# DIAGNijmegen/bodyct-dram-emph-subtype

Measured on AMD Instinct MI355X. Metric: CT volumes/sec (train step, 1x128x256x256), higher is better.
Workload: dtype f32; 1 GPU; BASELINE configs[1]: resnet18segcls train step (fwd+loss+bwd+Adam), batch 2/GPU, 1x128x256x256, fp32, inputs resident in HBM; global_batch=2, parallelism=dp1, hip_graph=False, streams=2

## Files before the change

### bodyct-dram-emph-subtype_amd/csrc/wino_gemm.hip

```cpp
#include <stdlib.h>
#include "wino_gemm.h"

namespace {

template <int MI, int NJ>
__device__ __forceinline__ void zero_acc(f32x16 (&acc)[MI][NJ]) {
#pragma unroll
  for (int mi = 0; mi < MI; ++mi)
#pragma unroll
    for (int nj = 0; nj < NJ; ++nj)
#pragma unroll
      for (int e = 0; e < 16; ++e) acc[mi][nj][e] = 0.f;
}


struct NnTile { const float* Ab; const float* Bb; float* Yb; int mt, nt; };
template <int NJ>
__device__ __forceinline__ NnTile nn_tile(const int idx, const float* A, const float* Bw, float* Y, const int N,
                                          const int K, const int m_tiles, const int n_tiles, const int nblk,
                                          const int npts) {
  constexpr int BN = 64 * NJ;
  const int L = xcd_remap(idx, nblk);
  NnTile t;
  t.nt = L % n_tiles;
// ... 252 lines not shown
            if (fused) {
              v += bv;
              if (ep.add) {
                const long oo = o - Y;
                const f32x4 av = *reinterpret_cast<const f32x4*>(ep.add + oo);
                if (ep.gate) {
                  const f32x4 gv = *reinterpret_cast<const f32x4*>(ep.gate + oo);
#pragma unroll
                  for (int j = 0; j < 4; ++j) v[j] += gv[j] > 0.f ? av[j] : 0.f;
                } else {
                  v += av;
                }
              }
#pragma unroll
              for (int j = 0; j < 4; ++j) { s1v[cr][j] += v[j]; s2v[cr][j] += v[j] * v[j]; }
            }
            *reinterpret_cast<f32x4*>(o) = v;
          }
        }
      }
    }
    if (ep.stats) {
#pragma unroll
      for (int cr = 0; cr < NR; ++cr)
#pragma unroll
        for (int j = 0; j < 4; ++j)
#pragma unroll
          for (int o = Q; o < 64; o <<= 1) {
            s1v[cr][j] += __shfl_xor(s1v[cr][j], o, 64);
            s2v[cr][j] += __shfl_xor(s2v[cr][j], o, 64);
          }
      __syncthreads();
      float* red = s1;
      if (rs == 0) {
#pragma unroll
        for (int cr = 0; cr < NR; ++cr)
#pragma unroll
          for (int j = 0; j < 4; ++j) {
            red[(ln.wave * 2 + 0) * 32 * NJ + cr * CW + 4 * cq + j] = s1v[cr][j];
            red[(ln.wave * 2 + 1) * 32 * NJ + cr * CW + 4 * cq + j] = s2v[cr][j];
          }
      }
      __syncthreads();
      if (ln.tid < 2 * BN) {
        const int which = ln.tid / BN, cc = ln.tid - which * BN;
        const int cwn = cc / (32 * NJ), c2 = cc - cwn * 32 * NJ;
        float v = 0.f;
#pragma unroll
        for (int w = 0; w < 4; ++w) v += red[((cwn * 4 + w) * 2 + which) * 32 * NJ + c2];
        ep.stats[((long)cur.mt * 2 + which) * N + cur.nt * BN + cc] = v;
      }
    }
    if (!more) break;
    idx = nxt;
    cur = nx;
  }
}
#ifndef DRAM_STREAM_NT
#define DRAM_STREAM_NT 2
#endif
template <int NJ, int KT, int S, bool DB = false, int KH = 1>
__global__ __launch_bounds__(256, DB ? 2 : 1) void wino_gemm_nn_stream_kernel(const float* __restrict__ A,
                                                                    const float* __restrict__ Bw, float* __restrict__ Y,
                                                                    const int npts, const int m64, const int per_wg,
                                                                    const int total) {
  constexpr int N = 64 * NJ;
  constexpr int STG = 64 * KT;
  constexpr int SPR = KT / 4;
  constexpr int RPI = 64 / SPR;
  constexpr int IPW = 64 / RPI / 4;
  constexpr int BPW = N / RPI / 4;
  constexpr int KG = KT / 8;
  constexpr int P = DB ? 40 : 32 * NJ + 8;
  constexpr int KS = KT * KH;
  static_assert(S == 3 || S == 4, "ring depth");
  static_assert(KH == 1 || (KH == 2 && DB && S == 3), "k halves: direct-B form, three stages");
  __shared__ __attribute__((aligned(1024))) float st0[STG], st1[STG], st2[STG], st3[S == 4 ? STG : 64];
  __shared__ __attribute__((aligned(1024))) float bt[DB ? 64 : N * KT];
  __shared__ __attribute__((aligned(16))) float turn[4 * 32 * P];

  const int tid = threadIdx.x, lane = tid & 63;
  const int wave = __builtin_amdgcn_readfirstlane(tid >> 6);
  const int li = lane & 31, lh = lane >> 5;
  const int i0 = blockIdx.x * per_wg;
  const int n = (i0 + per_wg <= total ? per_wg : total - i0);
  if (n <= 0) return;

  int aoff[IPW], boff[BPW];
#pragma unroll
  for (int j = 0; j < IPW; ++j) {
    const int row = RPI * (wave + 4 * j) + lane / SPR, ph = lane % SPR;
    aoff[j] = row * KS + ((ph & ~15) | ((ph ^ row) & 15)) * 4;
  }
#pragma unroll
  for (int j = 0; j < BPW; ++j) {
    const int row = RPI * (wave + 4 * j) + lane / SPR, ph = lane % SPR;
    boff[j] = row * KT + ((ph & ~15) | ((ph ^ row) & 15)) * 4;
  }
  auto a_src = [&](int item) __attribute__((always_inline)) {
    const int ti = item / KH, h = item - ti * KH;
    const int xi = ti / m64, t = ti - xi * m64;
    return A + (((long)(t >> 2) * npts + xi) * 256 + (t & 3) * 64) * KS + h * KT;
  };
  auto issue_a = [&](int item, float* stage) __attribute__((always_inline)) {
    const float* src = a_src(item);
#pragma unroll
    for (int j = 0; j < IPW; ++j)
      __builtin_amdgcn_global_load_lds((const __attribute__((address_space(1))) void*)(src + aoff[j]),
                                       (__attribute__((address_space(3))) void*)(stage + (wave + 4 * j) * 256), 16, 0,
                                       DRAM_STREAM_NT);
  };
  auto stage_of = [&](int k) __attribute__((always_inline)) -> float* {
    return k == 0 ? st0 : (k == 1 ? st1 : (k == 2 ? st2 : st3));
  };

  const int r0 = 32 * (wave & 1), c0 = 32 * NJ * (wave >> 1);
  const int arow = r0 + li;
  f32x4 bfr[NJ][KG * KH];
  auto load_b = [&](int xi) __attribute__((always_inline)) {
    if (DB) {
      const float* srcd = Bw + (long)xi * N * KS;
#pragma unroll
      for (int nj = 0; nj < NJ; ++nj)
#pragma unroll
        for (int kg = 0; kg < KG * KH; ++kg)
          bfr[nj][kg] = *reinterpret_cast<const f32x4*>(srcd + (c0 + nj * 32 + li) * KS + (2 * kg + lh) * 4);
      __builtin_amdgcn_s_waitcnt(0x0F70);
      asm volatile("" ::: "memory");
      return;
    }
    __syncthreads();
    const float* src = Bw + (long)xi * N * KT;
#pragma unroll
    for (int j = 0; j < BPW; ++j)
      __builtin_amdgcn_global_load_lds((const __attribute__((address_space(1))) void*)(src + boff[j]),
                                       (__attribute__((address_space(3))) void*)(bt + (wave + 4 * j) * 256), 16, 0, 0);
    __builtin_amdgcn_s_waitcnt(0x0F70);
    asm volatile("" ::: "memory");
    __syncthreads();
#pragma unroll
    for (int nj = 0; nj < NJ; ++nj) {
      const int brow = c0 + nj * 32 + li;
#pragma unroll
      for (int kg = 0; kg < KG; ++kg) {
        const int sl = 2 * kg + lh;
        bfr[nj][kg] = *reinterpret_cast<const f32x4*>(bt + brow * KT + ((sl & ~15) | ((sl ^ brow) & 15)) * 4);
      }
    }
  };

  int xi_cur = i0 / KH / m64;
#pragma unroll
  for (int k = 0; k < S - 1; ++k)
    if (k < n) issue_a(i0 + k, stage_of(k));
  load_b(xi_cur);

  float* reg = turn + wave * (32 * P);
  constexpr int Q = 8 * NJ;
  const int cq = lane % Q, rs = lane / Q;

  constexpr int U = S * KH;
  f32x16 acc[NJ];
  for (int itb = 0; itb < n; itb += U) {
#pragma unroll
    for (int k = 0; k < U; ++k) {
      const int it = itb + k;
      const int h = k % KH;
      if (it < n) {
        const int item = i0 + it;
        const int ti = item / KH;
        const int xi = ti / m64, t = ti - xi * m64;
        if (h == 0 && xi != xi_cur) {
          xi_cur = xi;
          load_b(xi);
        }
        if (it + S - 2 < n) __builtin_amdgcn_s_waitcnt(0x0F70 | ((IPW * (S - 2)) & 15) | (((IPW * (S - 2)) >> 4) << 14));
        else __builtin_amdgcn_s_waitcnt(0x0F70);
        asm volatile("" ::: "memory");
        __builtin_amdgcn_s_barrier();
        if (it + S - 1 < n) issue_a(item + S - 1, stage_of((k + S - 1) % S));
        const float* stg = stage_of(k % S);
        if (h == 0) {
#pragma unroll
          for (int nj = 0; nj < NJ; ++nj)
#pragma unroll
            for (int e = 0; e < 16; ++e) acc[nj][e] = 0.f;
        }
#pragma unroll
        for (int kg = 0; kg < KG; ++kg) {
          const int sl = 2 * kg + lh;
          const f32x4 af = *reinterpret_cast<const f32x4*>(stg + arow * KT + ((sl & ~15) | ((sl ^ arow) & 15)) * 4);
#pragma unroll
          for (int e = 0; e < 4; ++e)
#pragma unroll
            for (int nj = 0; nj < NJ; ++nj)
              acc[nj] = __builtin_amdgcn_mfma_f32_32x32x2f32(af[e], bfr[nj][h * KG + kg][e], acc[nj], 0, 0, 0);
        }
        if (h != KH - 1) continue;
        float* yb = Y + (((long)(t >> 2) * npts + xi) * 256 + (t & 3) * 64 + r0) * N + c0;
        if (DB) {
          const int cq8 = lane & 7, rs8 = lane >> 3;
#pragma unroll
          for (int nj = 0; nj < NJ; ++nj) {
#pragma unroll
            for (int e = 0; e < 16; ++e) reg[((e & 3) + 8 * (e >> 2) + 4 * lh) * P + li] = acc[nj][e];
#pragma unroll
            for (int r = 0; r < 4; ++r) {
              const int row = r * 8 + rs8;
              *reinterpret_cast<f32x4*>(yb + (long)row * N + nj * 32 + 4 * cq8) =
                  *reinterpret_cast<const f32x4*>(reg + row * P + 4 * cq8);
            }
          }
        } else {
#pragma unroll
          for (int e = 0; e < 16; ++e)
#pragma unroll
            for (int nj = 0; nj < NJ; ++nj) reg[((e & 3) + 8 * (e >> 2) + 4 * lh) * P + nj * 32 + li] = acc[nj][e];
#pragma unroll
          for (int r = 0; r < Q / 2; ++r) {
            const int row = r * (64 / Q) + rs;
            *reinterpret_cast<f32x4*>(yb + (long)row * N + 4 * cq) = *reinterpret_cast<const f32x4*>(reg + row * P + 4 * cq);
          }
        }
      }
    }
  }
}

typedef __bf16 bf16x8 __attribute__((ext_vector_type(8)));

template <int NJ, int NT>
__global__ __launch_bounds__(512) void wino_gemm_nn_bf16_kernel(const float* __restrict__ A, const float* __restrict__ Bw,
                                                                float* __restrict__ Y, const int Mpad, const int N,
                                                                const int K, const int m_tiles, const int n_tiles,
                                                                const int nblk, const int npts) {
  constexpr int STAGE = (256 + 64 * NJ) * 32;
  __shared__ __attribute__((aligned(1024))) float lds[2 * STAGE];
  const int tid = threadIdx.x;
  const int lane = tid & 63;
  const int wave = __builtin_amdgcn_readfirstlane(tid >> 6);
  const NnTile t = nn_tile<NJ>(blockIdx.x, A, Bw, Y, N, K, m_tiles, n_tiles, nblk, npts);
  const NnDma<NJ> dma(lane, wave, K);
  const int niter = K / 32;
  f32x16 acc[2][NJ];
  zero_acc(acc);

  const int li = lane & 31, lh = lane >> 5;
  const int wm = wave & 3, wn = wave >> 2;
  const int rsw = (li >> 1) & 7;
  const int a_row = (wm * 64 + li) * 32;
  const int b_row = 256 * 32 + (wn * NJ * 32 + li) * 32;

  dma.issue(t.Ab, t.Bb, 0, lds);
  for (int it = 0; it < niter; ++it) {
    __syncthreads();
    if (it + 1 < niter) dma.issue(t.Ab, t.Bb, it + 1, lds + ((it + 1) & 1) * STAGE);
    const float* st = lds + (it & 1) * STAGE;
#pragma unroll
    for (int j = 0; j < 2; ++j) {
      const int sh = ((2 * j + lh) ^ rsw) * 4, sl = ((4 + 2 * j + lh) ^ rsw) * 4;
      bf16x8 ah[2], al[2], bh[NJ], bl[NJ];
#pragma unroll
      for (int mi = 0; mi < 2; ++mi) {
        ah[mi] = *reinterpret_cast<const bf16x8*>(st + a_row + mi * 32 * 32 + sh);
        if (NT > 1) al[mi] = *reinterpret_cast<const bf16x8*>(st + a_row + mi * 32 * 32 + sl);
      }
#pragma unroll
      for (int nj = 0; nj < NJ; ++nj) {
        bh[nj] = *reinterpret_cast<const bf16x8*>(st + b_row + nj * 32 * 32 + sh);
        if (NT > 1) bl[nj] = *reinterpret_cast<const bf16x8*>(st + b_row + nj * 32 * 32 + sl);
      }
#pragma unroll
      for (int nj = 0; nj < NJ; ++nj)
#pragma unroll
        for (int mi = 0; mi < 2; ++mi) {
          if (NT > 1) {
            acc[mi][nj] = __builtin_amdgcn_mfma_f32_32x32x16_bf16(al[mi], bh[nj], acc[mi][nj], 0, 0, 0);
            acc[mi][nj] = __builtin_amdgcn_mfma_f32_32x32x16_bf16(ah[mi], bl[nj], acc[mi][nj], 0, 0, 0);
          }
          acc[mi][nj] = __builtin_amdgcn_mfma_f32_32x32x16_bf16(ah[mi], bh[nj], acc[mi][nj], 0, 0, 0);
        }
    }
  }

#pragma unroll
  for (int mi = 0; mi < 2; ++mi)
#pragma unroll
    for (int e = 0; e < 16; ++e) {
      const int row = wm * 64 + mi * 32 + (e & 3) + 8 * (e >> 2) + 4 * lh;
      float* o = t.Yb + (long)row * N + wn * NJ * 32 + li;
#pragma unroll
      for (int nj = 0; nj < NJ; ++nj) o[nj * 32] = acc[mi][nj][e];
    }
}

struct TnTile {
  int nt, mt, split, xi;
  int t0, t1;
  __device__ __forceinline__ long row(const int it, const int npts) const {
    const int tt = t0 + it * 32;
    return ((long)(tt >> 8) * npts + xi) * 256 + (tt & 255);
  }
};
__device__ __forceinline__ TnTile tn_tile(const int bid, const int nblk, const int m_tiles, const int n_tiles,
                                          const int nsplit, const int kper, const int Tpad) {
  int L = xcd_remap(bid, nblk);
  TnTile t;
  t.nt = L % n_tiles; L /= n_tiles;
  t.mt = L % m_tiles; L /= m_tiles;
  t.split = L % nsplit;
  t.xi = L / nsplit;
  t.t0 = t.split * kper;
  t.t1 = (t.t0 + kper < Tpad) ? t.t0 + kper : Tpad;
  return t;
}
template <int WMW, int MI, int NJ>
__global__ __launch_bounds__(512) void wino_gemm_tn_kernel(const float* __restrict__ Ah, const float* __restrict__ Bh,
                                                           float* __restrict__ slab, const int Tpad, const int M,
                                                           const int N, const int m_tiles, const int n_tiles,
                                                           const int nsplit, const int kper, const int nblk,
                                                           const int npts) {
  constexpr int WNW = 8 / WMW;
  constexpr int BM = WMW * 32 * MI, BN = WNW * 32 * NJ;
  static_assert(BM % 64 == 0 && BM <= 256 && BN % 64 == 0 && BN <= 256, "one DMA piece = 256 floats");
  constexpr int STAGE = 32 * (BM + BN);
  constexpr int AQ = BM / 4, ARPP = 64 / AQ, APW = BM / 64;
  constexpr int BQ = BN / 4, BRPP = 64 / BQ, BPW = BN / 64;
  __shared__ __attribute__((aligned(1024))) float lds[2 * STAGE];

  const int tid = threadIdx.x;
  const int lane = tid & 63;
  const int wave = __builtin_amdgcn_readfirstlane(tid >> 6);
  const TnTile t = tn_tile(blockIdx.x, nblk, m_tiles, n_tiles, nsplit, kper, Tpad);
  int bcol = t.nt * BN + (lane % BQ) * 4;
  if (bcol > N - 4) bcol = N - 4;
  const float* Ab = Ah + (long)(lane / AQ) * M + t.mt * BM + (lane % AQ) * 4;
  const float* Bb = Bh + (long)(lane / BQ) * N + bcol;

  auto issue = [&](int it, int stage) __attribute__((always_inline)) {
    float* as = lds + stage * STAGE;
    float* bs = as + 32 * BM;
    const long row = t.row(it, npts);
    const float* ag = Ab + row * M;
    const float* bg = Bb + row * N;
#pragma unroll
    for (int j = 0; j < APW; ++j) {
      const int p = APW * wave + j;
      __builtin_amdgcn_global_load_lds((const __attribute__((address_space(1))) void*)(ag + (long)(p * ARPP) * M),
                                       (__attribute__((address_space(3))) void*)(as + p * 256), 16, 0, 0);
    }
#pragma unroll
    for (int jj = 0; jj < BPW; ++jj) {
      const int p = BPW * wave + jj;
      __builtin_amdgcn_global_load_lds((const __attribute__((address_space(1))) void*)(bg + (long)(p * BRPP) * N),
                                       (__attribute__((address_space(3))) void*)(bs + p * 256), 16, 0, 0);
    }
  };

  f32x16 acc[MI][NJ];
  zero_acc(acc);

  const int li = lane & 31, lh = lane >> 5;
  const int wm = wave % WMW, wn = wave / WMW;
  const int niter = (t.t1 - t.t0) / 32;

  if (niter > 0) issue(0, 0);
  for (int it = 0; it < niter; ++it) {
    __syncthreads();
    if (it + 1 < niter) issue(it + 1, (it + 1) & 1);
    const float* as = lds + (it & 1) * STAGE + wm * 32 * MI + li;
    const float* bs = lds + (it & 1) * STAGE + 32 * BM + wn * 32 * NJ + li;
#pragma unroll 4
    for (int kk = 0; kk < 16; ++kk) {
      const int kr = 2 * kk + lh;
      float af[MI], bf[NJ];
#pragma unroll
      for (int mi = 0; mi < MI; ++mi) af[mi] = as[kr * BM + mi * 32];
#pragma unroll
      for (int nj = 0; nj < NJ; ++nj) bf[nj] = bs[kr * BN + nj * 32];
#pragma unroll
      for (int nj = 0; nj < NJ; ++nj)
#pragma unroll
        for (int mi = 0; mi < MI; ++mi)
          acc[mi][nj] = __builtin_amdgcn_mfma_f32_32x32x2f32(af[mi], bf[nj], acc[mi][nj], 0, 0, 0);
    }
  }

  float* sb = slab + (((long)t.split * npts + t.xi) * M + t.mt * BM) * N + t.nt * BN;
#pragma unroll
  for (int mi = 0; mi < MI; ++mi)
#pragma unroll
    for (int e = 0; e < 16; ++e) {
      const int row = wm * 32 * MI + mi * 32 + (e & 3) + 8 * (e >> 2) + 4 * lh;
      float* o = sb + (long)row * N + wn * 32 * NJ + li;
#pragma unroll
      for (int nj = 0; nj < NJ; ++nj)
        if (t.nt * BN + wn * 32 * NJ + nj * 32 + li < N) o[nj * 32] = acc[mi][nj][e];
    }
}

__global__ __launch_bounds__(512, 2) void wino_gemm_tn64_kernel(const float* __restrict__ Ah, const float* __restrict__ Bh,
                                                                float* __restrict__ slab, const int Tpad, const int nsplit,
                                                                const int kper, const int nblk, const int npts) {
  constexpr int M = 64, N = 64, KS = 64;
  constexpr int STAGE = KS * (M + N);
  __shared__ __attribute__((aligned(1024))) float lds[2 * STAGE];
  const int tid = threadIdx.x, lane = tid & 63;
  const int wave = __builtin_amdgcn_readfirstlane(tid >> 6);
  int L = xcd_remap(blockIdx.x, nblk);
  const int split = L % nsplit;
  const int xi = L / nsplit;
  const int t0 = split * kper;
  const int t1 = (t0 + kper < Tpad) ? t0 + kper : Tpad;
  const int prow = lane >> 4, pcol = (lane & 15) * 4;
  auto issue = [&](int it, int stage) __attribute__((always_inline)) {
    float* as = lds + stage * STAGE;
    float* bs = as + KS * M;
    const int tt = t0 + it * KS;
    const long row = ((long)(tt >> 8) * npts + xi) * 256 + (tt & 255);
#pragma unroll
    for (int j = 0; j < 2; ++j) {
      const int p = 2 * wave + j;
      __builtin_amdgcn_global_load_lds((const __attribute__((address_space(1))) void*)(Ah + (row + p * 4 + prow) * M + pcol),
                                       (__attribute__((address_space(3))) void*)(as + p * 256), 16, 0, 0);
      __builtin_amdgcn_global_load_lds((const __attribute__((address_space(1))) void*)(Bh + (row + p * 4 + prow) * N + pcol),
                                       (__attribute__((address_space(3))) void*)(bs + p * 256), 16, 0, 0);
    }
  };
  f32x16 acc;
#pragma unroll
  for (int e = 0; e < 16; ++e) acc[e] = 0.f;
  const int li = lane & 31, lh = lane >> 5;
  const int wm = wave & 1, wn = (wave >> 1) & 1, kh = wave >> 2;
  const int niter = (t1 - t0) / KS;
  if (niter > 0) issue(0, 0);
  for (int it = 0; it < niter; ++it) {
    __syncthreads();
    if (it + 1 < niter) issue(it + 1, (it + 1) & 1);
    const float* as = lds + (it & 1) * STAGE + (kh * 32) * M + wm * 32 + li;
    const float* bs = lds + (it & 1) * STAGE + KS * M + (kh * 32) * N + wn * 32 + li;
#pragma unroll 4
    for (int kk = 0; kk < 16; ++kk) {
      const int kr = 2 * kk + lh;
      acc = __builtin_amdgcn_mfma_f32_32x32x2f32(as[kr * M], bs[kr * N], acc, 0, 0, 0);
    }
  }
  __syncthreads();
  float* ex = lds + (wave & 3) * 1024;
  if (kh == 1) {
#pragma unroll
    for (int e = 0; e < 16; ++e) ex[e * 64 + lane] = acc[e];
  }
  __syncthreads();
  if (kh == 0) {
    float* sb = slab + (((long)split * npts + xi) * M) * N;
#pragma unroll
    for (int e = 0; e < 16; ++e) {
      const int row = wm * 32 + (e & 3) + 8 * (e >> 2) + 4 * lh;
      sb[(long)row * N + wn * 32 + li] = acc[e] + ex[e * 64 + lane];
    }
  }
}

typedef short s16x4 __attribute__((ext_vector_type(4)));
typedef short s16x8 __attribute__((ext_vector_type(8)));

template <int WMW, int MI, int NJ, int NT>
__global__ __launch_bounds__(512) void wino_gemm_tn_bf16_kernel(const float* __restrict__ Ah, const float* __restrict__ Bh,
                                                                float* __restrict__ slab, const int Tpad, const int M,
                                                                const int N, const int m_tiles, const int n_tiles,
                                                                const int nsplit, const int kper, const int nblk,
                                                                const int npts) {
  constexpr int WNW = 8 / WMW;
  constexpr int BM = WMW * 32 * MI, BN = WNW * 32 * NJ;
  static_assert(BM % 64 == 0 && BM <= 256 && BN % 64 == 0 && BN <= 256, "one DMA piece = 256 floats");
  constexpr int STAGE = 32 * (BM + BN);
  constexpr int AQ = BM / 4, ARPP = 64 / AQ, APW = BM / 64;
  constexpr int BQ = BN / 4, BRPP = 64 / BQ, BPW = BN / 64;
  __shared__ __attribute__((aligned(1024))) float lds[2 * STAGE];

  const int tid = threadIdx.x;
  const int lane = tid & 63;
  const int wave = __builtin_amdgcn_readfirstlane(tid >> 6);
  const TnTile t = tn_tile(blockIdx.x, nblk, m_tiles, n_tiles, nsplit, kper, Tpad);

  int acol[APW], bcol[BPW];
#pragma unroll
  for (int j = 0; j < APW; ++j) {
    const int r3 = (j * ARPP + lane / AQ) & 3, slot = lane % AQ;
    acol[j] = t.mt * BM + ((((slot >> 2) ^ r3) << 2) | (slot & 3)) * 4;
  }
#pragma unroll
  for (int j = 0; j < BPW; ++j) {
    const int r3 = (j * BRPP + lane / BQ) & 3, slot = lane % BQ;
    int c = t.nt * BN + ((((slot >> 2) ^ r3) << 2) | (slot & 3)) * 4;
    bcol[j] = c > N - 4 ? N - 4 : c;
  }
  const float* Ab = Ah + (long)(lane / AQ) * M;
  const float* Bb = Bh + (long)(lane / BQ) * N;

  auto issue = [&](int it, int stage) __attribute__((always_inline)) {
    float* as = lds + stage * STAGE;
    float* bs = as + 32 * BM;
    const long row = t.row(it, npts);
    const float* ag = Ab + row * M;
    const float* bg = Bb + row * N;
#pragma unroll
    for (int j = 0; j < APW; ++j) {
      const int p = APW * wave + j;
      __builtin_amdgcn_global_load_lds((const __attribute__((address_space(1))) void*)(ag + (long)(p * ARPP) * M + acol[j]),
                                       (__attribute__((address_space(3))) void*)(as + p * 256), 16, 0, 0);
    }
#pragma unroll
    for (int jj = 0; jj < BPW; ++jj) {
      const int p = BPW * wave + jj;
      __builtin_amdgcn_global_load_lds((const __attribute__((address_space(1))) void*)(bg + (long)(p * BRPP) * N + bcol[jj]),
                                       (__attribute__((address_space(3))) void*)(bs + p * 256), 16, 0, 0);
    }
  };

  f32x16 acc[MI][NJ];
  zero_acc(acc);

  const int li = lane & 31, lh = lane >> 5;
  const int wm = wave % WMW, wn = wave / WMW;
  const int niter = (t.t1 - t.t0) / 32;

  const int g4 = lane >> 4, q = (lane >> 2) & 3, p4 = lane & 3;
  const int rrow = (g4 >> 1) * 8 + q;
  const int cbyte = (g4 & 1) * 32 + p4 * 8;
  int a_hi[MI], a_lo[MI], b_hi[NJ], b_lo[NJ];
#pragma unroll
  for (int mi = 0; mi < MI; ++mi) {
    const int ch = 2 * (wm * MI + mi);
    a_hi[mi] = rrow * BM * 4 + ((ch ^ q) * 64) + cbyte;
    a_lo[mi] = rrow * BM * 4 + (((ch + 1) ^ q) * 64) + cbyte;
  }
#pragma unroll
  for (int nj = 0; nj < NJ; ++nj) {
    const int ch = 2 * (wn * NJ + nj);
    b_hi[nj] = 32 * BM * 4 + rrow * BN * 4 + ((ch ^ q) * 64) + cbyte;
    b_lo[nj] = 32 * BM * 4 + rrow * BN * 4 + (((ch + 1) ^ q) * 64) + cbyte;
  }
  auto frag = [&](const char* st, int off, int rstride) __attribute__((always_inline)) {
    const s16x4 r0 = __builtin_amdgcn_ds_read_tr16_b64_v4i16((__attribute__((address_space(3))) s16x4*)(st + off));
    const s16x4 r1 =
        __builtin_amdgcn_ds_read_tr16_b64_v4i16((__attribute__((address_space(3))) s16x4*)(st + off + 4 * rstride));
    return __builtin_bit_cast(bf16x8, __builtin_shufflevector(r0, r1, 0, 1, 2, 3, 4, 5, 6, 7));
  };

  if (niter > 0) issue(0, 0);
  for (int it = 0; it < niter; ++it) {
    __syncthreads();
    if (it + 1 < niter) issue(it + 1, (it + 1) & 1);
    const char* st = reinterpret_cast<const char*>(lds + (it & 1) * STAGE);
#pragma unroll
    for (int s16 = 0; s16 < 2; ++s16) {
      bf16x8 ah[MI], al[MI], bh[NJ], bl[NJ];
#pragma unroll
      for (int mi = 0; mi < MI; ++mi) {
        ah[mi] = frag(st, a_hi[mi] + s16 * 16 * BM * 4, BM * 4);
        if (NT > 1) al[mi] = frag(st, a_lo[mi] + s16 * 16 * BM * 4, BM * 4);
      }
#pragma unroll
      for (int nj = 0; nj < NJ; ++nj) {
        bh[nj] = frag(st, b_hi[nj] + s16 * 16 * BN * 4, BN * 4);
        if (NT > 1) bl[nj] = frag(st, b_lo[nj] + s16 * 16 * BN * 4, BN * 4);
      }
#pragma unroll
      for (int nj = 0; nj < NJ; ++nj)
#pragma unroll
        for (int mi = 0; mi < MI; ++mi) {
          if (NT > 1) {
            acc[mi][nj] = __builtin_amdgcn_mfma_f32_32x32x16_bf16(al[mi], bh[nj], acc[mi][nj], 0, 0, 0);
            acc[mi][nj] = __builtin_amdgcn_mfma_f32_32x32x16_bf16(ah[mi], bl[nj], acc[mi][nj], 0, 0, 0);
          }
          acc[mi][nj] = __builtin_amdgcn_mfma_f32_32x32x16_bf16(ah[mi], bh[nj], acc[mi][nj], 0, 0, 0);
        }
    }
  }

  float* sb = slab + (((long)t.split * npts + t.xi) * M + t.mt * BM) * N + t.nt * BN;
#pragma unroll
  for (int mi = 0; mi < MI; ++mi)
#pragma unroll
    for (int e = 0; e < 16; ++e) {
      const int row = wm * 32 * MI + mi * 32 + (e & 3) + 8 * (e >> 2) + 4 * lh;
      float* o = sb + (long)row * N + wn * 32 * NJ + li;
#pragma unroll
      for (int nj = 0; nj < NJ; ++nj)
        if (t.nt * BN + wn * 32 * NJ + nj * 32 + li < N) o[nj * 32] = acc[mi][nj][e];
    }
}

__global__ __launch_bounds__(256) void slab_sum_kernel(const float* __restrict__ slab, float* __restrict__ out, const long n,
                                                       const int nsplit) {
  __shared__ float part[4][64];
  const int r = threadIdx.x & 63, kg = threadIdx.x >> 6;
  for (long i0 = blockIdx.x * 64L; i0 < n; i0 += (long)gridDim.x * 64L) {
    const long i = i0 + r;
    const bool live = i < n;
    float p[8];
#pragma unroll
    for (int j = 0; j < 8; ++j) p[j] = 0.f;
    if (live) {
      int k = kg;
      for (; k + 28 < nsplit; k += 32) {
#pragma unroll
        for (int j = 0; j < 8; ++j) p[j] += slab[(long)(k + 4 * j) * n + i];
      }
      for (int j = 0; k < nsplit; k += 4, ++j) p[j] += slab[(long)k * n + i];
    }
    part[kg][r] = ((p[0] + p[1]) + (p[2] + p[3])) + ((p[4] + p[5]) + (p[6] + p[7]));
    __syncthreads();
    if (kg == 0 && live) out[i] = (part[0][r] + part[1][r]) + (part[2][r] + part[3][r]);
    __syncthreads();
  }
}
}


bool plan_tn(const DramConvDesc* d, const WinoGeom& g, TnPlan& p) {
  const int M = d->Cout, N = d->Cin;
  p.bm = M % 256 == 0 ? 256 : (M % 128 == 0 ? 128 : 64);
  const int ncand = p.bm == 256 ? 3 : 2;
  const int cand[3] = {256, 128, 64};
  p.bn = 0;
  int best_pad = 1 << 30;
  for (int i = 0; i < ncand; ++i) {
    const int padded = (N + cand[i] - 1) / cand[i] * cand[i];
    if (padded * 100 <= N * 113) { p.bn = cand[i]; break; }
    if (padded < best_pad) { best_pad = padded; p.bn = cand[i]; }
  }
  p.m_tiles = M / p.bm;
  p.n_tiles = (N + p.bn - 1) / p.bn;
  if (p.bn >= 128 && (p.bn > 128 || p.bm == 256)) {
    const long w1 = (long)g.npts * p.m_tiles * p.n_tiles;
    const int hb = p.bn / 2, hn = (N + hb - 1) / hb;
    const long w2 = (long)g.npts * p.m_tiles * hn;
    if (w1 >= 512 && (double)((w2 + 255) / 256) * 0.5 * 1.03 < (double)((w1 + 255) / 256)) {
      p.bn = hb;
      p.n_tiles = hn;
    }
  }
  const int base = g.npts * p.m_tiles * p.n_tiles;
  const int k32 = g.Tpad / 32;
  int ns = 1;
  while (base * ns < (g.npts == 1 ? 256 : 512) && ns * 2 <= k32 / 4 && ns < (g.npts == 1 ? 256 : 16)) ns *= 2;
  p.nsplit = ns;
  p.kper = ((k32 + ns - 1) / ns) * 32;
  return true;
}

int run_nn(const float* A, const float* U, float* Y, const WinoGeom& g, int N, int K, hipStream_t s,
           const GemmEpilogue ep, const int math, const bool alone) {
  const int m_tiles = g.Tpad / 256;
  int nj = 1;
  double best = 1e30;
  for (int c = 4; c >= 1; c >>= 1) {
    if (N % (64 * c) != 0) continue;
    const long wgs = (long)g.npts * m_tiles * (N / (64 * c));
    const double cost = (double)((wgs + 255) / 256) * c * (c == 4 ? 1.0 : (c == 2 ? 1.03 : 1.10));
    if (cost < best) { best = cost; nj = c; }
  }
  const int n_tiles = N / (64 * nj);
  const int nblk = g.npts * m_tiles * n_tiles;
  DramProf prof(DRAM_FAM_WINO_GEMM_NN, nj, 2.0 * g.npts * (double)g.Tpad * N * K,
                4.0 * g.npts * ((double)g.Tpad * (K + N) + (double)N * K), s,
                g.npts > 1 ? 2.0 * g.B * g.D * g.H * g.W * (double)N * K * 27.0 : -1.0);
  if (math) {
#define WNB(NJ_, NT_)                                                                                                  \
  hipLaunchKernelGGL((wino_gemm_nn_bf16_kernel<NJ_, NT_>), dim3(nblk), dim3(512), 0, s, A, U, Y, g.Tpad, N, K, m_tiles, \
                     n_tiles, nblk, g.npts)
    if (math == 1) { if (nj == 4) WNB(4, 3); else if (nj == 2) WNB(2, 3); else WNB(1, 3); }
    else { if (nj == 4) WNB(4, 1); else if (nj == 2) WNB(2, 1); else WNB(1, 1); }
#undef WNB
    DRAM_LAUNCH_CHECK();
    return DRAM_OK;
  }
#define WNN(NJ_)                                                                                                   \
  hipLaunchKernelGGL((wino_gemm_nn_kernel<NJ_>), dim3(nblk), dim3(512), 0, s, A, U, Y, g.Tpad, N, K, m_tiles, n_tiles, \
                     nblk, g.npts, ep)
  const char* se = tune_env("DRAM_NN_STREAM");
  const int stream_on = se ? atoi(se) : 1;
  const bool fused = ep.bias || ep.add || ep.gate || ep.stats;
  if (stream_on && !fused && g.npts > 1 && g.Tpad % 256 == 0 &&
      ((N == 64 && (K == 128 || K == 64)) || (N == 128 && K == 64))) {
    const int m64 = g.Tpad / 64;
    const long total = (long)g.npts * m64;
    if (total < (1L << 31) && (total >= 4096 || stream_on == 2)) {
      const int wgs = stream_on == 2 ? 8 : 256;
      const int per_wg = (int)((total + wgs - 1) / wgs);
      const int grid = (int)((total + per_wg - 1) / per_wg);
#define WNS(NJ_, KT_, S_)                                                                                          \
  hipLaunchKernelGGL((wino_gemm_nn_stream_kernel<NJ_, KT_, S_>), dim3(grid), dim3(256), 0, s, A, U, Y, g.npts, m64, \
                     per_wg, (int)total)
      const char* sde = tune_env("DRAM_NN_STREAM_DB");
      const int sdb = sde ? atoi(sde) : (alone ? 7 : 0);
      const int wgs2 = stream_on == 2 ? 8 : 512;
      const int per2 = (int)((total + wgs2 - 1) / wgs2);
      const int grid2 = (int)((total + per2 - 1) / per2);
      if (N == 64 && K == 128 && (sdb & 4)) {
        const long total2 = 2 * total;
        if (total2 < (1L << 31)) {
          const int perk = 2 * (int)((total + wgs2 - 1) / wgs2);
          const int gridk = (int)((total2 + perk - 1) / perk);
          hipLaunchKernelGGL((wino_gemm_nn_stream_kernel<1, 64, 3, true, 2>), dim3(gridk), dim3(256), 0, s, A, U, Y, g.npts,
                             m64, perk, (int)total2);
        } else WNS(1, 128, 3);
      }
      else if (N == 64 && K == 128) WNS(1, 128, 3);
      else if (N == 64 && (sdb & 1))
        hipLaunchKernelGGL((wino_gemm_nn_stream_kernel<1, 64, 3, true>), dim3(grid2), dim3(256), 0, s, A, U, Y, g.npts, m64,
                           per2, (int)total);
      else if (N == 128 && (sdb & 2))
        hipLaunchKernelGGL((wino_gemm_nn_stream_kernel<2, 64, 3, true>), dim3(grid2), dim3(256), 0, s, A, U, Y, g.npts, m64,
                           per2, (int)total);
      else if (N == 64) WNS(1, 64, 4);
      else WNS(2, 64, 4);
#undef WNS
      DRAM_LAUNCH_CHECK();
      return DRAM_OK;
    }
  }
  const char* pe = tune_env("DRAM_NN_PERSIST");
  const int persist = pe ? atoi(pe) : 1;
  if (persist && !fused && nj <= 2 && (K / 32) % 2 == 0) {
    const int rounds = (nblk + 255) / 256;
    int grid = ((nblk + rounds - 1) / rounds + 7) / 8 * 8;
    if (grid > 256) grid = 256;
    if (grid > nblk) grid = nblk;
#define WNP(NJ_)                                                                                                   \
  hipLaunchKernelGGL((wino_gemm_nn_pers_kernel<NJ_>), dim3(grid), dim3(512), 0, s, A, U, Y, g.Tpad, N, K, m_tiles, \
                     n_tiles, nblk, g.npts, ep)
    if (nj == 2) WNP(2);
    else WNP(1);
#undef WNP
    DRAM_LAUNCH_CHECK();
    return DRAM_OK;
  }
  if (nj == 4) WNN(4);
  else if (nj == 2) WNN(2);
  else WNN(1);
#undef WNN
  DRAM_LAUNCH_CHECK();
  return DRAM_OK;
}

int run_tn(const float* Ah, const float* Bh, float* slab, const WinoGeom& g, const TnPlan& p, const int M, const int N,
           const int math, hipStream_t s) {
  const int nblk = g.npts * p.nsplit * p.m_tiles * p.n_tiles;
  DramProf prof(DRAM_FAM_WINO_GEMM_TN, p.bm * 1000 + p.bn, 2.0 * g.npts * (double)g.Tpad * M * N,
                4.0 * g.npts * ((double)g.Tpad * (M + N) + (double)p.nsplit * M * N), s,
                g.npts > 1 ? 2.0 * g.B * g.D * g.H * g.W * (double)M * N * 27.0 : -1.0);
  auto launch = [&](auto kernel) {
    hipLaunchKernelGGL(kernel, dim3(nblk), dim3(512), 0, s, Ah, Bh, slab, g.Tpad, M, N, p.m_tiles, p.n_tiles, p.nsplit,
                       p.kper, nblk, g.npts);
  };
#define WTN(WM_, MI_, NJ_)                                             \
  launch(math == 1   ? wino_gemm_tn_bf16_kernel<WM_, MI_, NJ_, 3>      \
         : math == 2 ? wino_gemm_tn_bf16_kernel<WM_, MI_, NJ_, 1>      \
                     : wino_gemm_tn_kernel<WM_, MI_, NJ_>)
  if (math == 0 && g.npts > 1 && M == 64 && N == 64 && p.kper % 64 == 0 && g.Tpad % 64 == 0)
    hipLaunchKernelGGL(wino_gemm_tn64_kernel, dim3(g.npts * p.nsplit), dim3(512), 0, s, Ah, Bh, slab, g.Tpad, p.nsplit,
                       p.kper, g.npts * p.nsplit, g.npts);
  else if (p.bm == 256 && p.bn == 256) WTN(4, 2, 4);
  else if (p.bm == 256 && p.bn == 128) WTN(4, 2, 2);
  else if (p.bm == 256 && p.bn == 64) WTN(4, 2, 1);
  else if (p.bm == 128 && p.bn == 256) WTN(2, 2, 2);
  else if (p.bm == 128 && p.bn == 128) WTN(2, 2, 1);
  else if (p.bm == 64 && p.bn == 256) WTN(2, 1, 2);
  else if (p.bm == 64 && p.bn == 128) WTN(2, 1, 1);
  else return DRAM_ERR_UNSUPPORTED;
#undef WTN
  DRAM_LAUNCH_CHECK();
  return DRAM_OK;
}

namespace {
bool c1_ok(const DramConvDesc* d) {
  if (!d || d->k != 1 || d->stride != 1 || d->pad != 0) return false;
  if (d->B < 1 || d->D < 1 || d->H < 1 || d->W < 1) return false;
  if (d->Do != d->D || d->Ho != d->H || d->Wo != d->W) return false;
  if (d->Cin < 64 || d->Cout < 64 || d->Cin % 64 != 0 || d->Cout % 64 != 0) return false;
  const long long M = (long long)d->B * d->D * d->H * d->W;
  const long long cmax = d->Cin > d->Cout ? d->Cin : d->Cout;
  return M % 256 == 0 && M * cmax < (1LL << 31);
}
WinoGeom c1_geom(const DramConvDesc* d) {
  WinoGeom g{};
  g.B = d->B; g.D = d->D; g.H = d->H; g.W = d->W; g.d = 1;
  g.nz = g.ny = g.nx = 1;
  g.npts = 1;
  g.T = g.Tpad = d->B * d->D * d->H * d->W;
  return g;
}
}

extern "C" int dram_conv1x1_applicable(const DramConvDesc* d) { return c1_ok(d) ? 1 : 0; }

extern "C" int dram_conv1x1_num_stat_rows(const DramConvDesc* d) {
  if (!c1_ok(d)) return DRAM_ERR_UNSUPPORTED;
  return c1_geom(d).Tpad / 256;
}

extern "C" int dram_conv1x1_fwd(const float* x, const float* w2d, const float* bias, float* y, float* stats_partial,
                                const DramConvDesc* d, dram_stream_t stream) {
  if (!x || !w2d || !y) return DRAM_ERR_BAD_ARG;
  if (!c1_ok(d)) return DRAM_ERR_UNSUPPORTED;
  return run_nn(x, w2d, y, c1_geom(d), d->Cout, d->Cin, (hipStream_t)stream,
                GemmEpilogue{bias, nullptr, nullptr, stats_partial});
}

extern "C" int dram_conv1x1_bwd_data(const float* dy, const float* wt, float* dx, const float* add, const float* gate,
                                     const DramConvDesc* d, dram_stream_t stream) {
  if (!dy || !wt || !dx || (gate && !add)) return DRAM_ERR_BAD_ARG;
  if (!c1_ok(d)) return DRAM_ERR_UNSUPPORTED;
  return run_nn(dy, wt, dx, c1_geom(d), d->Cin, d->Cout, (hipStream_t)stream, GemmEpilogue{nullptr, add, gate, nullptr});
}

extern "C" size_t dram_conv1x1_bwd_weight_workspace(const DramConvDesc* d) {
  if (!c1_ok(d)) return 0;
  TnPlan p;
  plan_tn(d, c1_geom(d), p);
  return (size_t)p.nsplit * d->Cout * d->Cin * sizeof(float);
}

extern "C" int dram_conv1x1_bwd_weight(const float* x, const float* dy, float* dw, const DramConvDesc* d, void* workspace,
                                       size_t workspace_bytes, dram_stream_t stream) {
  if (!x || !dy || !dw) return DRAM_ERR_BAD_ARG;
  if (!c1_ok(d)) return DRAM_ERR_UNSUPPORTED;
  const WinoGeom g = c1_geom(d);
  TnPlan p;
  plan_tn(d, g, p);
  const size_t need = (size_t)p.nsplit * d->Cout * d->Cin * sizeof(float);
  if (p.nsplit > 1 && (!workspace || workspace_bytes < need)) return DRAM_ERR_WORKSPACE;
  hipStream_t s = (hipStream_t)stream;
  float* slab = p.nsplit > 1 ? (float*)workspace : dw;
  const int rc = run_tn(dy, x, slab, g, p, d->Cout, d->Cin, 0, s);
  if (rc != DRAM_OK) return rc;
  if (p.nsplit > 1) {
    const long n = (long)d->Cout * d->Cin;
    const int grid = (int)((n + 63) / 64 > 4096 ? 4096 : (n + 63) / 64);
    DramProf prof(DRAM_FAM_WINO_WGRAD_OUT, 0, 0.0, 4.0 * (double)n * (p.nsplit + 1), s);
    hipLaunchKernelGGL(slab_sum_kernel, dim3(grid), dim3(256), 0, s, slab, dw, n, p.nsplit);
    DRAM_LAUNCH_CHECK();
  }
  return DRAM_OK;
}
```

Baseline: 55.15 volumes/sec.

## Add persistent and streaming ring-buffered TN Winograd GEMM kernels for weight gradients

Adds two fp32 TN GEMM variants for the Winograd weight-gradient path. The first is a persistent kernel in which each workgroup processes several tiles and prefetches the next tile's first K-slice while finishing the current one. The second is a streaming kernel specialised for M=64,N=128 that keeps a 3-deep LDS ring filled by global_load_lds with explicit waitcnt. Both are enabled by default through an env knob and aim to cut launch/tail underutilisation and memory latency stalls, at the cost of extra kernel complexity and possibly lower occupancy or less parallelism for some shapes.

```diff
diff --git a/bodyct-dram-emph-subtype_amd/csrc/wino_gemm.hip b/bodyct-dram-emph-subtype_amd/csrc/wino_gemm.hip
--- a/bodyct-dram-emph-subtype_amd/csrc/wino_gemm.hip
+++ b/bodyct-dram-emph-subtype_amd/csrc/wino_gemm.hip
@@ -578,9 +578,8 @@
     return ((long)(tt >> 8) * npts + xi) * 256 + (tt & 255);
   }
 };
-__device__ __forceinline__ TnTile tn_tile(const int bid, const int nblk, const int m_tiles, const int n_tiles,
-                                          const int nsplit, const int kper, const int Tpad) {
-  int L = xcd_remap(bid, nblk);
+__device__ __forceinline__ TnTile tn_item(int L, const int m_tiles, const int n_tiles, const int nsplit, const int kper,
+                                          const int Tpad) {
   TnTile t;
   t.nt = L % n_tiles; L /= n_tiles;
   t.mt = L % m_tiles; L /= m_tiles;
@@ -589,6 +588,10 @@
   t.t0 = t.split * kper;
   t.t1 = (t.t0 + kper < Tpad) ? t.t0 + kper : Tpad;
   return t;
+}
+__device__ __forceinline__ TnTile tn_tile(const int bid, const int nblk, const int m_tiles, const int n_tiles,
+                                          const int nsplit, const int kper, const int Tpad) {
+  return tn_item(xcd_remap(bid, nblk), m_tiles, n_tiles, nsplit, kper, Tpad);
 }
 template <int WMW, int MI, int NJ>
 __global__ __launch_bounds__(512) void wino_gemm_tn_kernel(const float* __restrict__ Ah, const float* __restrict__ Bh,
@@ -734,6 +737,208 @@
     for (int e = 0; e < 16; ++e) {
       const int row = wm * 32 + (e & 3) + 8 * (e >> 2) + 4 * lh;
       sb[(long)row * N + wn * 32 + li] = acc[e] + ex[e * 64 + lane];
+    }
+  }
+}
+
+template <int WMW, int MI, int NJ>
+__global__ __launch_bounds__(512) void wino_gemm_tn_pers_kernel(const float* __restrict__ Ah, const float* __restrict__ Bh,
+                                                                float* __restrict__ slab, const int Tpad, const int M,
+                                                                const int N, const int m_tiles, const int n_tiles,
+                                                                const int nsplit, const int kper, const int nblk,
+                                                                const int npts, const int per_wg) {
+  constexpr int WNW = 8 / WMW;
+  constexpr int BM = WMW * 32 * MI, BN = WNW * 32 * NJ;
+  static_assert(BM % 64 == 0 && BM <= 256 && BN % 64 == 0 && BN <= 256, "one DMA piece = 256 floats");
+  constexpr int AQ = BM / 4, ARPP = 64 / AQ, APW = BM / 64;
+  constexpr int BQ = BN / 4, BRPP = 64 / BQ, BPW = BN / 64;
+  __shared__ __attribute__((aligned(1024))) float a0[32 * BM], a1[32 * BM];
+  __shared__ __attribute__((aligned(1024))) float b0[32 * BN], b1[32 * BN];
+
+  const int tid = threadIdx.x;
+  const int lane = tid & 63;
+  const int wave = __builtin_amdgcn_readfirstlane(tid >> 6);
+  const int li = lane & 31, lh = lane >> 5;
+  const int wm = wave % WMW, wn = wave / WMW;
+  const int first = xcd_remap(blockIdx.x, gridDim.x) * per_wg;
+  const int last = first + per_wg < nblk ? first + per_wg : nblk;
+  if (first >= last) return;
+  const int niter = kper / 32;
+
+  auto a_src = [&](const TnTile& t) __attribute__((always_inline)) {
+    return Ah + (long)(lane / AQ) * M + t.mt * BM + (lane % AQ) * 4;
+  };
+  auto b_src = [&](const TnTile& t) __attribute__((always_inline)) {
+    int bcol = t.nt * BN + (lane % BQ) * 4;
+    if (bcol > N - 4) bcol = N - 4;
+    return Bh + (long)(lane / BQ) * N + bcol;
+  };
+  auto issue = [&](const TnTile& t, const float* Ab, const float* Bb, int it, float* as, float* bs)
+      __attribute__((always_inline)) {
+    const long row = t.row(it, npts);
+    const float* ag = Ab + row * M;
+    const float* bg = Bb + row * N;
+#pragma unroll
+    for (int j = 0; j < APW; ++j) {
+      const int p = APW * wave + j;
+      __builtin_amdgcn_global_load_lds((const __attribute__((address_space(1))) void*)(ag + (long)(p * ARPP) * M),
+                                       (__attribute__((address_space(3))) void*)(as + p * 256), 16, 0, 0);
+    }
+#pragma unroll
+    for (int jj = 0; jj < BPW; ++jj) {
+      const int p = BPW * wave + jj;
+      __builtin_amdgcn_global_load_lds((const __attribute__((address_space(1))) void*)(bg + (long)(p * BRPP) * N),
+                                       (__attribute__((address_space(3))) void*)(bs + p * 256), 16, 0, 0);
+    }
+  };
+  f32x16 acc[MI][NJ];
+  auto kstep = [&](const float* sa, const float* sb) __attribute__((always_inline)) {
+    const float* as = sa + wm * 32 * MI + li;
+    const float* bs = sb + wn * 32 * NJ + li;
+#pragma unroll 4
+    for (int kk = 0; kk < 16; ++kk) {
+      const int kr = 2 * kk + lh;
+      float af[MI], bf[NJ];
+#pragma unroll
+      for (int mi = 0; mi < MI; ++mi) af[mi] = as[kr * BM + mi * 32];
+#pragma unroll
+      for (int nj = 0; nj < NJ; ++nj) bf[nj] = bs[kr * BN + nj * 32];
+#pragma unroll
+      for (int nj = 0; nj < NJ; ++nj)
+#pragma unroll
+        for (int mi = 0; mi < MI; ++mi)
+          acc[mi][nj] = __builtin_amdgcn_mfma_f32_32x32x2f32(af[mi], bf[nj], acc[mi][nj], 0, 0, 0);
+    }
+  };
+
+  int idx = first;
+  TnTile cur = tn_item(idx, m_tiles, n_tiles, nsplit, kper, Tpad);
+  const float* Ab = a_src(cur);
+  const float* Bb = b_src(cur);
+  issue(cur, Ab, Bb, 0, a0, b0);
+  for (;;) {
+    const bool more = idx + 1 < last;
+    TnTile nx = cur;
+    if (more) nx = tn_item(idx + 1, m_tiles, n_tiles, nsplit, kper, Tpad);
+    const float* nAb = a_src(nx);
+    const float* nBb = b_src(nx);
+    zero_acc(acc);
+    for (int it = 0; it < niter; it += 2) {
+      __syncthreads();
+      issue(cur, Ab, Bb, it + 1, a1, b1);
+      kstep(a0, b0);
+      __syncthreads();
+      if (it + 2 < niter) issue(cur, Ab, Bb, it + 2, a0, b0);
+      else if (more) issue(nx, nAb, nBb, 0, a0, b0);
+      kstep(a1, b1);
+    }
+    float* sb = slab + (((long)cur.split * npts + cur.xi) * M + cur.mt * BM) * N + cur.nt * BN;
+#pragma unroll
+    for (int mi = 0; mi < MI; ++mi)
+#pragma unroll
+      for (int e = 0; e < 16; ++e) {
+        const int row = wm * 32 * MI + mi * 32 + (e & 3) + 8 * (e >> 2) + 4 * lh;
+        float* o = sb + (long)row * N + wn * 32 * NJ + li;
+#pragma unroll
+        for (int nj = 0; nj < NJ; ++nj)
+          if (cur.nt * BN + wn * 32 * NJ + nj * 32 + li < N) o[nj * 32] = acc[mi][nj][e];
+      }
+    if (!more) break;
+    ++idx;
+    cur = nx;
+    Ab = nAb;
+    Bb = nBb;
+  }
+}
+
+template <int S>
+__global__ __launch_bounds__(256, 4) void wino_gemm_tn_stream_kernel(const float* __restrict__ Ah, const float* __restrict__ Bh,
+                                                                     float* __restrict__ slab, const int Tpad,
+                                                                     const int nsplit, const int kper, const int nchains,
+                                                                     const int npts) {
+  constexpr int M = 64, N = 128, R = 16;
+  constexpr int IPW = 3;
+  static_assert(S == 3 || S == 4, "ring depth");
+  __shared__ __attribute__((aligned(1024))) float sa0[R * M], sa1[R * M], sa2[R * M], sa3[S == 4 ? R * M : 64];
+  __shared__ __attribute__((aligned(1024))) float sb0[R * N], sb1[R * N], sb2[R * N], sb3[S == 4 ? R * N : 64];
+
+  const int tid = threadIdx.x, lane = tid & 63;
+  const int wave = __builtin_amdgcn_readfirstlane(tid >> 6);
+  const int li = lane & 31, lh = lane >> 5;
+  const int wm = wave & 1, wn = wave >> 1;
+  const int a_lane = (lane >> 4) * M + (lane & 15) * 4;
+  const int b_lane = (lane >> 5) * N + (lane & 31) * 4;
+  auto a_of = [&](int k) __attribute__((always_inline)) -> float* {
+    return k == 0 ? sa0 : (k == 1 ? sa1 : (k == 2 ? sa2 : sa3));
+  };
+  auto b_of = [&](int k) __attribute__((always_inline)) -> float* {
+    return k == 0 ? sb0 : (k == 1 ? sb1 : (k == 2 ? sb2 : sb3));
+  };
+
+  for (int c = blockIdx.x; c < nchains; c += gridDim.x) {
+    const int L = xcd_remap(c, nchains);
+    const int split = L % nsplit, xi = L / nsplit;
+    const int t0 = split * kper;
+    const int t1 = (t0 + kper < Tpad) ? t0 + kper : Tpad;
+    const int n = t1 > t0 ? (t1 - t0) / R : 0;
+    auto issue = [&](int s, float* sa, float* sb) __attribute__((always_inline)) {
+      const int g = t0 + R * s + 4 * wave;
+      const long row = ((long)(g >> 8) * npts + xi) * 256 + (g & 255);
+      __builtin_amdgcn_global_load_lds((const __attribute__((address_space(1))) void*)(Ah + row * M + a_lane),
+                                       (__attribute__((address_space(3))) void*)(sa + wave * 256), 16, 0, 0);
+#pragma unroll
+      for (int j = 0; j < 2; ++j)
+        __builtin_amdgcn_global_load_lds((const __attribute__((address_space(1))) void*)(Bh + (row + 2 * j) * N + b_lane),
+                                         (__attribute__((address_space(3))) void*)(sb + (2 * wave + j) * 256), 16, 0, 0);
+    };
+    __builtin_amdgcn_s_waitcnt(0x0F70);
+    asm volatile("" ::: "memory");
+    __builtin_amdgcn_s_barrier();
+    if (n > 0) issue(0, a_of(S - 1), b_of(S - 1));
+#pragma unroll
+    for (int k = 0; k < S - 1; ++k)
+      if (k < n) issue(k, a_of(k), b_of(k));
+
+    f32x16 acc[2];
+#pragma unroll
+    for (int a = 0; a < 2; ++a)
+#pragma unroll
+      for (int e = 0; e < 16; ++e) acc[a][e] = 0.f;
+
+    auto stage = [&](const int k, const int it, const bool full) __attribute__((always_inline)) {
+      if (full || it + S - 2 < n) __builtin_amdgcn_s_waitcnt(0x0F70 | (IPW * (S - 2)));
+      else __builtin_amdgcn_s_waitcnt(0x0F70);
+      asm volatile("" ::: "memory");
+      __builtin_amdgcn_s_barrier();
+      if (full || it + S - 1 < n) issue(it + S - 1, a_of((k + S - 1) % S), b_of((k + S - 1) % S));
+      const float* as = a_of(k) + wm * 32 + li;
+      const float* bs = b_of(k) + wn * 64 + li;
+#pragma unroll
+      for (int kk = 0; kk < R / 2; ++kk) {
+        const int kr = 2 * kk + lh;
+        const float af = as[kr * M], b0 = bs[kr * N], b1 = bs[kr * N + 32];
+        acc[0] = __builtin_amdgcn_mfma_f32_32x32x2f32(af, b0, acc[0], 0, 0, 0);
+        acc[1] = __builtin_amdgcn_mfma_f32_32x32x2f32(af, b1, acc[1], 0, 0, 0);
+      }
+    };
+    int itb = 0;
+    for (; itb + 2 * S - 2 < n; itb += S) {
+#pragma unroll
+      for (int k = 0; k < S; ++k) stage(k, itb + k, true);
+    }
+    for (; itb < n; itb += S) {
+#pragma unroll
+      for (int k = 0; k < S; ++k)
+        if (itb + k < n) stage(k, itb + k, false);
+    }
+
+    float* sb = slab + (((long)split * npts + xi) * M) * N;
+#pragma unroll
+    for (int e = 0; e < 16; ++e) {
+      const int row = wm * 32 + (e & 3) + 8 * (e >> 2) + 4 * lh;
+      float* o = sb + (long)row * N + wn * 64 + li;
+      o[0] = acc[0][e];
+      o[32] = acc[1][e];
     }
   }
 }
@@ -1037,6 +1242,47 @@
   launch(math == 1   ? wino_gemm_tn_bf16_kernel<WM_, MI_, NJ_, 3>      \
          : math == 2 ? wino_gemm_tn_bf16_kernel<WM_, MI_, NJ_, 1>      \
                      : wino_gemm_tn_kernel<WM_, MI_, NJ_>)
+  const char* te = tune_env("DRAM_NN_STREAM");
+  const int tn_stream = te ? atoi(te) : 1;
+  if (math == 0 && tn_stream) {
+    const bool t64 = g.npts > 1 && M == 64 && N == 64 && p.kper % 64 == 0 && g.Tpad % 64 == 0;
+    if (g.npts > 1 && M == 64 && N == 128 && p.bm == 64 && p.bn == 128) {
+      const int nchains = g.npts * p.nsplit;
+      const int grid = tn_stream == 2 && nchains > 8 ? 8 : nchains;
+      hipLaunchKernelGGL((wino_gemm_tn_stream_kernel<3>), dim3(grid), dim3(256), 0, s, Ah, Bh, slab, g.Tpad, p.nsplit, p.kper,
+                         nchains, g.npts);
+      DRAM_LAUNCH_CHECK();
+      return DRAM_OK;
+    }
+    const int niter = p.kper / 32;
+    const bool whole = niter % 2 == 0 && (long)p.kper * p.nsplit == g.Tpad;
+    if (!t64 && whole && (tn_stream == 2 || (g.npts > 1 && niter <= 4))) {
+      const int slots = 256 * (p.bm + p.bn <= 256 ? 2 : 1);
+      const int rounds = (nblk + slots - 1) / slots;
+      int grid = ((nblk + rounds - 1) / rounds + 7) / 8 * 8;
+      if (grid > slots) grid = slots;
+      if (tn_stream == 2) grid = 8;
+      if (grid > nblk) grid = nblk;
+      const int per_wg = (nblk + grid - 1) / grid;
+      grid = (nblk + per_wg - 1) / per_wg;
+      if (per_wg > 1 || tn_stream == 2) {
+#define WTP(WM_, MI_, NJ_)                                                                                              \
+  hipLaunchKernelGGL((wino_gemm_tn_pers_kernel<WM_, MI_, NJ_>), dim3(grid), dim3(512), 0, s, Ah, Bh, slab, g.Tpad, M, N, \
+                     p.m_tiles, p.n_tiles, p.nsplit, p.kper, nblk, g.npts, per_wg)
+        if (p.bm == 256 && p.bn == 256) WTP(4, 2, 4);
+        else if (p.bm == 256 && p.bn == 128) WTP(4, 2, 2);
+        else if (p.bm == 256 && p.bn == 64) WTP(4, 2, 1);
+        else if (p.bm == 128 && p.bn == 256) WTP(2, 2, 2);
+        else if (p.bm == 128 && p.bn == 128) WTP(2, 2, 1);
+        else if (p.bm == 64 && p.bn == 256) WTP(2, 1, 2);
+        else if (p.bm == 64 && p.bn == 128) WTP(2, 1, 1);
+        else return DRAM_ERR_UNSUPPORTED;
+#undef WTP
+        DRAM_LAUNCH_CHECK();
+        return DRAM_OK;
+      }
+    }
+  }
   if (math == 0 && g.npts > 1 && M == 64 && N == 64 && p.kper % 64 == 0 && g.Tpad % 64 == 0)
     hipLaunchKernelGGL(wino_gemm_tn64_kernel, dim3(g.npts * p.nsplit), dim3(512), 0, s, Ah, Bh, slab, g.Tpad, p.nsplit,
                        p.kper, g.npts * p.nsplit, g.npts);
```

New measurement: 55.75 volumes/sec (median of 6 runs). 1.01x the previous value.
